# GLAD-RUC/FastEGNN

Measured on AMD Instinct MI355X. Metric: graphs/sec (fwd+bwd), Water-3D-like 100k-node frame, higher is better.
Workload: dtype f32; 1 GPU; cfg4 Water-3D-like frame (SURVEY 8d): uniform points, radius graph r=0.035 (mean degree ~19), gravity on; 4-layer FastEGNN H=64, fwd+loss+bwd, CSR build inside the step; nodes=100000, edges=1919172, graphs_per_batch=1, virtual_channels=16, layers=4, parallelism=1 GPU, launch=whole step replayed as one captured HIP graph

## Files before the change

### fastegnn_amd/csrc/common.h

```cpp
#pragma once
#include <hip/hip_runtime.h>
#include <stdint.h>

namespace fe {

typedef float f32x4 __attribute__((ext_vector_type(4)));

constexpr int H = 64;
constexpr int QXLD = 68;
constexpr int TS = 68;
constexpr int IMG = 4096;
constexpr int FEATW = 8;

struct Vec {
  f32x4 t[4];
};

__device__ __forceinline__ int lane_id() { return threadIdx.x & 63; }
__device__ __forceinline__ int wave_id() { return __builtin_amdgcn_readfirstlane((int)(threadIdx.x >> 6)); }
__device__ __forceinline__ int global_wave_id() { return (int)(blockIdx.x * (blockDim.x >> 6)) + wave_id(); }

__device__ __forceinline__ float sigmoid_f(float z) { return __builtin_amdgcn_rcpf(1.0f + __expf(-z)); }
__device__ __forceinline__ float silu_f(float z) { return z * sigmoid_f(z); }
__device__ __forceinline__ float dsilu_f(float z) {
// ... 399 lines not shown
  for (int p = 0; p < 3; ++p) fr[0][p] = ip[p * 512];
  __builtin_amdgcn_sched_group_barrier(0x100, 3, 0);
#pragma unroll
  for (int g = 0; g < 8; ++g) {
    const int s = g >> 2, t = g & 3, cb = g & 1;
    if (g + 1 < 8) {
      const int sn = (g + 1) >> 2, tn = (g + 1) & 3;
#pragma unroll
      for (int p = 0; p < 3; ++p) fr[cb ^ 1][p] = ip[p * 512 + (tn * 2 + sn) * 64];
      __builtin_amdgcn_sched_group_barrier(0x100, 3, 0);
    }
    const bf16x8 ah = __builtin_bit_cast(bf16x8, fr[cb][0]), am = __builtin_bit_cast(bf16x8, fr[cb][1]),
                 al = __builtin_bit_cast(bf16x8, fr[cb][2]);
    const bf16x8 xh = __builtin_bit_cast(bf16x8, in.p[0][s]);
    const bf16x8 xm = __builtin_bit_cast(bf16x8, in.p[1][s]);
    const bf16x8 xl = __builtin_bit_cast(bf16x8, in.p[2][s]);
    acc.t[t] = __builtin_amdgcn_mfma_f32_16x16x32_bf16(al, xh, acc.t[t], 0, 0, 0);
    acc.t[t] = __builtin_amdgcn_mfma_f32_16x16x32_bf16(am, xm, acc.t[t], 0, 0, 0);
    acc.t[t] = __builtin_amdgcn_mfma_f32_16x16x32_bf16(ah, xl, acc.t[t], 0, 0, 0);
    acc.t[t] = __builtin_amdgcn_mfma_f32_16x16x32_bf16(am, xh, acc.t[t], 0, 0, 0);
    acc.t[t] = __builtin_amdgcn_mfma_f32_16x16x32_bf16(ah, xm, acc.t[t], 0, 0, 0);
    acc.t[t] = __builtin_amdgcn_mfma_f32_16x16x32_bf16(ah, xh, acc.t[t], 0, 0, 0);
    __builtin_amdgcn_sched_group_barrier(0x008, 6, 0);
  }
  __builtin_amdgcn_sched_barrier(0);
#endif
}
__device__ __forceinline__ void gemm64_x3(const unsigned *img3, const Vec &in, Vec &acc) { gemm64_x3(img3, vsplit(in), acc); }

__device__ __forceinline__ void gemm64_x3_t2(const unsigned *img3, const Vec &v, Vec &acc) {
  const u32x4 *ip = reinterpret_cast<const u32x4 *>(img3) + lane_id();
#pragma unroll
  for (int s = 0; s < 2; ++s) {
    float x[8];
    u32x4 ph, pm;
#pragma unroll
    for (int e = 0; e < 8; ++e) x[e] = v.t[2 * s + (e >> 2)][e & 3];
#pragma unroll
    for (int w = 0; w < 4; ++w) {
      ph[w] = part_pack(x[2 * w], x[2 * w + 1]);
      pm[w] = part_pack(x[2 * w], x[2 * w + 1]);
    }
    const bf16x8 xh = __builtin_bit_cast(bf16x8, ph), xm = __builtin_bit_cast(bf16x8, pm);
#pragma unroll
    for (int t = 0; t < 4; ++t) {
      const bf16x8 ah = __builtin_bit_cast(bf16x8, ip[(t * 2 + s) * 64]);
      const bf16x8 am = __builtin_bit_cast(bf16x8, ip[512 + (t * 2 + s) * 64]);
      const bf16x8 al = __builtin_bit_cast(bf16x8, ip[1024 + (t * 2 + s) * 64]);
      acc.t[t] = __builtin_amdgcn_mfma_f32_16x16x32_bf16(al, xh, acc.t[t], 0, 0, 0);
      acc.t[t] = __builtin_amdgcn_mfma_f32_16x16x32_bf16(am, xm, acc.t[t], 0, 0, 0);
      acc.t[t] = __builtin_amdgcn_mfma_f32_16x16x32_bf16(am, xh, acc.t[t], 0, 0, 0);
      acc.t[t] = __builtin_amdgcn_mfma_f32_16x16x32_bf16(ah, xm, acc.t[t], 0, 0, 0);
      acc.t[t] = __builtin_amdgcn_mfma_f32_16x16x32_bf16(ah, xh, acc.t[t], 0, 0, 0);
    }
  }
}

typedef float f32x2 __attribute__((ext_vector_type(2)));
typedef __bf16 bf16x2 __attribute__((ext_vector_type(2)));
__device__ __forceinline__ unsigned pack_rne(float x0, float x1) {
  return __builtin_bit_cast(unsigned, __builtin_convertvector(f32x2{x0, x1}, bf16x2));
}
__device__ __forceinline__ float round_bf(float x) { return (float)(__bf16)x; }
__host__ __device__ __forceinline__ float round_bf_host(float x) {
  unsigned u = __builtin_bit_cast(unsigned, x);
  u = (u + 0x7fffu + ((u >> 16) & 1u)) & 0xffff0000u;
  return __builtin_bit_cast(float, u);
}
struct BfOp {
  u32x4 p[2];
};
__device__ __forceinline__ BfOp vpack_bf(const Vec &v) {
  BfOp B;
#pragma unroll
  for (int s = 0; s < 2; ++s)
#pragma unroll
    for (int w = 0; w < 4; ++w) {
      const int e = 2 * w;
      B.p[s][w] = pack_rne(v.t[2 * s + (e >> 2)][e & 3], v.t[2 * s + ((e + 1) >> 2)][(e + 1) & 3]);
    }
  return B;
}
__device__ __forceinline__ Vec vround(const Vec &v) { return vmap(v, [](float z) { return round_bf(z); }); }
__device__ __forceinline__ void gemm64_b1(const unsigned *img3, const BfOp &in, Vec &acc) {
  const u32x4 *ip = reinterpret_cast<const u32x4 *>(img3) + lane_id();
#pragma unroll
  for (int s = 0; s < 2; ++s) {
    const bf16x8 x = __builtin_bit_cast(bf16x8, in.p[s]);
#pragma unroll
    for (int t = 0; t < 4; ++t)
      acc.t[t] = __builtin_amdgcn_mfma_f32_16x16x32_bf16(__builtin_bit_cast(bf16x8, ip[(t * 2 + s) * 64]), x, acc.t[t], 0, 0, 0);
  }
}

constexpr int RM_RS = 144;
constexpr int RM_PART = 64 * RM_RS;
constexpr int RM_BYTES = 3 * RM_PART;
constexpr int RM_WORDS = RM_BYTES / 4;
typedef unsigned u32x2 __attribute__((ext_vector_type(2)));
typedef short s16x4 __attribute__((ext_vector_type(4)));
__device__ __forceinline__ u32x2 lds_tr_read(const char *p) {
  return __builtin_bit_cast(u32x2, __builtin_amdgcn_ds_read_tr16_b64_v4i16(
                                       (__attribute__((address_space(3))) s16x4 *)(p)));
}
template <bool TR>
__device__ __forceinline__ bf16x8 rm_frag(const char *img, int part, int t, int s) {
  const int l = lane_id(), i = l & 15, q = l >> 4;
  u32x2 lo, hi;
  if constexpr (TR) {
    const char *p = img + part * RM_PART + (32 * s + 4 * q + (i >> 2)) * RM_RS + (16 * t + 4 * (i & 3)) * 2;
    lo = lds_tr_read(p);
    hi = lds_tr_read(p + 16 * RM_RS);
  } else {
    const char *p = img + part * RM_PART + (16 * t + i) * RM_RS + (32 * s + 4 * q) * 2;
#ifdef FE_RM_READ2
    lo = *reinterpret_cast<const u32x2 *>(p);
    hi = *reinterpret_cast<const u32x2 *>(p + 32);
#else
    typedef __attribute__((address_space(3))) const volatile u32x2 *lds_vu32x2;
    lo = *(lds_vu32x2)(p);
    hi = *(lds_vu32x2)(p + 32);
#endif
  }
  return __builtin_bit_cast(bf16x8, u32x4{lo[0], lo[1], hi[0], hi[1]});
}
template <bool TR, bool PIPE = true>
__device__ __forceinline__ void gemm64_x3_rm(const char *img, const Split &in, Vec &acc) {
#ifdef FE_NO_GEMM_PIPE
  constexpr bool pipe = false;
#else
  constexpr bool pipe = PIPE;
#endif
  if constexpr (!pipe) {
#pragma unroll
  for (int s = 0; s < 2; ++s)
#pragma unroll
    for (int t = 0; t < 4; ++t) {
      const bf16x8 ah = rm_frag<TR>(img, 0, t, s), am = rm_frag<TR>(img, 1, t, s), al = rm_frag<TR>(img, 2, t, s);
      const bf16x8 xh = __builtin_bit_cast(bf16x8, in.p[0][s]);
      const bf16x8 xm = __builtin_bit_cast(bf16x8, in.p[1][s]);
      const bf16x8 xl = __builtin_bit_cast(bf16x8, in.p[2][s]);
      acc.t[t] = __builtin_amdgcn_mfma_f32_16x16x32_bf16(al, xh, acc.t[t], 0, 0, 0);
      acc.t[t] = __builtin_amdgcn_mfma_f32_16x16x32_bf16(am, xm, acc.t[t], 0, 0, 0);
      acc.t[t] = __builtin_amdgcn_mfma_f32_16x16x32_bf16(ah, xl, acc.t[t], 0, 0, 0);
      acc.t[t] = __builtin_amdgcn_mfma_f32_16x16x32_bf16(am, xh, acc.t[t], 0, 0, 0);
      acc.t[t] = __builtin_amdgcn_mfma_f32_16x16x32_bf16(ah, xm, acc.t[t], 0, 0, 0);
      acc.t[t] = __builtin_amdgcn_mfma_f32_16x16x32_bf16(ah, xh, acc.t[t], 0, 0, 0);
    }
  } else {
  __builtin_amdgcn_sched_barrier(0);
  bf16x8 fr[2][3];
#pragma unroll
  for (int p = 0; p < 3; ++p) fr[0][p] = rm_frag<TR>(img, p, 0, 0);
  __builtin_amdgcn_sched_group_barrier(0x100, 6, 0);
#pragma unroll
  for (int g = 0; g < 8; ++g) {
    const int s = g >> 2, t = g & 3, cb = g & 1;
    if (g + 1 < 8) {
#pragma unroll
      for (int p = 0; p < 3; ++p) fr[cb ^ 1][p] = rm_frag<TR>(img, p, (g + 1) & 3, (g + 1) >> 2);
      __builtin_amdgcn_sched_group_barrier(0x100, 6, 0);
    }
    const bf16x8 ah = fr[cb][0], am = fr[cb][1], al = fr[cb][2];
    const bf16x8 xh = __builtin_bit_cast(bf16x8, in.p[0][s]);
    const bf16x8 xm = __builtin_bit_cast(bf16x8, in.p[1][s]);
    const bf16x8 xl = __builtin_bit_cast(bf16x8, in.p[2][s]);
// ... 586 lines not shown
```

### fastegnn_amd/csrc/misc.hip

```cpp
#include <cstdlib>
#include "kernels.h"

namespace fe {

__global__ void embed_fwd_kernel(const float *nf, int N, int nfd, const float *W, const float *b, float *h) {
  long idx = (long)blockIdx.x * blockDim.x + threadIdx.x;
  if (idx >= (long)N * H) return;
  int n = (int)(idx >> 6), o = (int)(idx & 63);
  float acc = b[o];
  for (int a = 0; a < nfd; ++a) acc += nf[(size_t)n * nfd + a] * W[o * nfd + a];
  h[idx] = acc;
}
__global__ void dgrad_small_kernel(const float *G, long N, int kf, const float *W, int ldw, int c0, float *g_in, int accumulate) {
  long idx = (long)blockIdx.x * blockDim.x + threadIdx.x;
  if (idx >= N * kf) return;
  long n = idx / kf;
  int a = (int)(idx % kf);
  float acc = 0.f;
  for (int o = 0; o < H; ++o) acc += G[(size_t)n * H + o] * W[(size_t)o * ldw + c0 + a];
  g_in[idx] = accumulate ? g_in[idx] + acc : acc;
}

__global__ void virtual_init_kernel(const float *vnf, int B, int C, float *HvT) {
  long idx = (long)blockIdx.x * blockDim.x + threadIdx.x;
// ... 146 lines not shown
      for (int ti = 0; ti < 4; ++ti) {
        if (want_bias && !rnd) bsum[ti] += av[ti];
#pragma unroll
        for (int tk = 0; tk < 4; ++tk)
          acc[ti][tk] = __builtin_amdgcn_mfma_f32_16x16x4f32(av[ti], bv[tk], acc[ti][tk], 0, 0, 0);
      }
    }
  }
}

#ifndef FE_WG_DEPTH
#define FE_WG_DEPTH 2
#endif
__device__ __forceinline__ void wg_accumulate_direct(const float *G, const float *T, int ldg, int ldt, long m_first, long m1,
                                                     int step, bool want_bias, bool rnd, f32x4 (&acc)[4][4], float (&bsum)[4]) {
  constexpr int D = FE_WG_DEPTH;
  const int l = lane_id(), i = l & 15, k = l >> 4;
  float gv[D][16], tv[D][16];
  unsigned og[4], ot[4];
#pragma unroll
  for (int s = 0; s < 4; ++s) {
    og[s] = ((unsigned)(4 * s + k) * (unsigned)ldg + (unsigned)i) * 4u;
    ot[s] = ((unsigned)(4 * s + k) * (unsigned)ldt + (unsigned)i) * 4u;
  }
  auto issue = [&](int slot, long m) {
    const char *gb = reinterpret_cast<const char *>(G + (size_t)m * ldg);
    const char *tb = reinterpret_cast<const char *>(T + (size_t)m * ldt);
    const bool full = m + 16 <= m1;
#pragma unroll
    for (int s = 0; s < 4; ++s) {
      const bool ok = full || m + 4 * s + k < m1;
      const unsigned a = ok ? og[s] : (unsigned)i * 4u, b = ok ? ot[s] : (unsigned)i * 4u;
#pragma unroll
      for (int t = 0; t < 4; ++t) {
        gv[slot][4 * s + t] = *reinterpret_cast<const float *>(gb + a + 64u * t);
        tv[slot][4 * s + t] = *reinterpret_cast<const float *>(tb + b + 64u * t);
      }
    }
  };
  auto consume = [&](int slot, long m) {
    const bool full = m + 16 <= m1;
#pragma unroll
    for (int s = 0; s < 4; ++s) {
      float av[4], bv[4];
      const bool ok = full || m + 4 * s + k < m1;
#pragma unroll
      for (int t = 0; t < 4; ++t) {
        av[t] = ok ? gv[slot][4 * s + t] : 0.f;
        bv[t] = ok ? tv[slot][4 * s + t] : 0.f;
      }
      if (rnd) {
#pragma unroll
        for (int t = 0; t < 4; ++t) {
          if (want_bias) bsum[t] += av[t];
          av[t] = round_bf(av[t]);
          bv[t] = round_bf(bv[t]);
        }
      }
#pragma unroll
      for (int ti = 0; ti < 4; ++ti) {
        if (want_bias && !rnd) bsum[ti] += av[ti];
#pragma unroll
        for (int tk = 0; tk < 4; ++tk)
          acc[ti][tk] = __builtin_amdgcn_mfma_f32_16x16x4f32(av[ti], bv[tk], acc[ti][tk], 0, 0, 0);
      }
    }
  };
  long m = m_first;
#pragma unroll
  for (int d = 0; d < D; ++d)
    if (m + (long)d * step < m1) issue(d, m + (long)d * step);
  while (m < m1) {
#pragma unroll
    for (int d = 0; d < D; ++d) {
      if (m < m1) {
        consume(d, m);
        if (m + (long)D * step < m1) issue(d, m + (long)D * step);
        m += step;
      }
    }
  }
}

struct WgParts { u32x4 p[3]; };
template <bool BF>
__device__ __forceinline__ WgParts wg_split8(const float (&x)[8]) {
  WgParts P;
  if constexpr (BF) {
#pragma unroll
    for (int w = 0; w < 4; ++w) P.p[0][w] = pack_rne(x[2 * w], x[2 * w + 1]);
    P.p[1] = P.p[2] = u32x4{0u, 0u, 0u, 0u};
  } else {
    float y[8];
#pragma unroll
    for (int e = 0; e < 8; ++e) y[e] = x[e];
#pragma unroll
    for (int w = 0; w < 4; ++w) {
      P.p[0][w] = part_pack(y[2 * w], y[2 * w + 1]);
      P.p[1][w] = part_pack(y[2 * w], y[2 * w + 1]);
      P.p[2][w] = part_pack(y[2 * w], y[2 * w + 1]);
    }
  }
  return P;
}
template <bool BF>
__device__ __forceinline__ void wg_accumulate_x3(const float *G, const float *T, int ldg, int ldt, long m_first, long m1,
                                                 int step, bool want_bias, f32x4 (&acc)[4][4], float (&bsum)[4]) {
  const int l = lane_id(), i = l & 15, q = l >> 4;
  float gr[4][8], tr[4][8];
  unsigned og[8], ot[8];
#pragma unroll
  for (int e = 0; e < 8; ++e) {
    og[e] = ((unsigned)(8 * q + e) * (unsigned)ldg + (unsigned)i) * 4u;
    ot[e] = ((unsigned)(8 * q + e) * (unsigned)ldt + (unsigned)i) * 4u;
  }
  auto load_g = [&](long m) {
    const char *gb = reinterpret_cast<const char *>(G + (size_t)m * ldg);
    const bool full = m + 32 <= m1;
#pragma unroll
    for (int e = 0; e < 8; ++e) {
      const unsigned a = (full || m + 8 * q + e < m1) ? og[e] : (unsigned)i * 4u;
#pragma unroll
      for (int t = 0; t < 4; ++t) gr[t][e] = *reinterpret_cast<const float *>(gb + a + 64u * t);
    }
  };
  auto load_t = [&](long m, int t) {
    const char *tb = reinterpret_cast<const char *>(T + (size_t)m * ldt);
    const bool full = m + 32 <= m1;
#pragma unroll
    for (int e = 0; e < 8; ++e) {
      const unsigned a = (full || m + 8 * q + e < m1) ? ot[e] : (unsigned)i * 4u;
      tr[t][e] = *reinterpret_cast<const float *>(tb + a + 64u * t);
    }
  };
  long m = m_first;
  if (m < m1) {
    load_g(m);
#pragma unroll
    for (int t = 0; t < 4; ++t) load_t(m, t);
  }
  for (; m < m1; m += step) {
    const bool full = m + 32 <= m1;
    const bool more = m + step < m1;
    WgParts gp[4];
#pragma unroll
    for (int t = 0; t < 4; ++t) {
      if (!full) {
#pragma unroll
        for (int e = 0; e < 8; ++e)
          if (m + 8 * q + e >= m1) gr[t][e] = 0.f;
      }
      if (want_bias) {
#pragma unroll
        for (int e = 0; e < 8; ++e) bsum[t] += gr[t][e];
      }
      gp[t] = wg_split8<BF>(gr[t]);
    }
    if (more) load_g(m + step);
#pragma unroll
    for (int tk = 0; tk < 4; ++tk) {
      if (!full) {
#pragma unroll
        for (int e = 0; e < 8; ++e)
          if (m + 8 * q + e >= m1) tr[tk][e] = 0.f;
      }
      const WgParts tp = wg_split8<BF>(tr[tk]);
      if (more) load_t(m + step, tk);
      const bf16x8 bh = __builtin_bit_cast(bf16x8, tp.p[0]), bm = __builtin_bit_cast(bf16x8, tp.p[1]),
                   bl = __builtin_bit_cast(bf16x8, tp.p[2]);
#pragma unroll
      for (int ti = 0; ti < 4; ++ti) {
        const bf16x8 ah = __builtin_bit_cast(bf16x8, gp[ti].p[0]);
        if constexpr (BF) {
          acc[ti][tk] = __builtin_amdgcn_mfma_f32_16x16x32_bf16(ah, bh, acc[ti][tk], 0, 0, 0);
        } else {
          const bf16x8 am = __builtin_bit_cast(bf16x8, gp[ti].p[1]), al = __builtin_bit_cast(bf16x8, gp[ti].p[2]);
          acc[ti][tk] = __builtin_amdgcn_mfma_f32_16x16x32_bf16(al, bh, acc[ti][tk], 0, 0, 0);
          acc[ti][tk] = __builtin_amdgcn_mfma_f32_16x16x32_bf16(am, bm, acc[ti][tk], 0, 0, 0);
          acc[ti][tk] = __builtin_amdgcn_mfma_f32_16x16x32_bf16(ah, bl, acc[ti][tk], 0, 0, 0);
          acc[ti][tk] = __builtin_amdgcn_mfma_f32_16x16x32_bf16(am, bh, acc[ti][tk], 0, 0, 0);
          acc[ti][tk] = __builtin_amdgcn_mfma_f32_16x16x32_bf16(ah, bm, acc[ti][tk], 0, 0, 0);
          acc[ti][tk] = __builtin_amdgcn_mfma_f32_16x16x32_bf16(ah, bh, acc[ti][tk], 0, 0, 0);
        }
      }
    }
  }
}

__global__ __launch_bounds__(256, FE_WG_OCC) void wgrad_tn_kernel(WgTable tab) {
#if defined(FE_WG_STAGED)
  __shared__ __attribute__((aligned(16))) float smem[4 * 2 * 16 * WTS];
#else
  __shared__ __attribute__((aligned(16))) float smem[4 * IMG];
#endif
  __shared__ float redb[H];
  float *red = smem;
  int jb = 0;
#pragma unroll 1
  while (jb + 1 < tab.n_jobs && (int)blockIdx.x >= tab.job[jb + 1].wg_begin) ++jb;
  const WgJob &a = tab.job[jb];
  const int local = blockIdx.x - a.wg_begin;
  int bidx = local % a.nb, split = local / a.nb;
#ifdef FE_WG_XCD
  if (a.nb > 1 && (a.nsplit & 7) == 0 && (a.wg_begin & 7) == 0) {
    const int xcd = local & 7, slot = local >> 3;
    bidx = slot % a.nb;
    split = xcd + 8 * (slot / a.nb);
  }
#endif
  const int l = lane_id(), i = l & 15, q = l >> 4, w = wave_id();
  const float *G = a.G + (size_t)bidx * a.sG;
  const float *T = a.T + (size_t)bidx * a.sT;
  const long m0 = (long)split * a.rows_per_wg;
  long m1 = m0 + a.rows_per_wg;
  if (m1 > a.M) m1 = a.M;
  if (threadIdx.x < H) redb[threadIdx.x] = 0.f;
  float *gt = smem + (w * 2 + 0) * 16 * WTS, *tt = smem + (w * 2 + 1) * 16 * WTS;
  f32x4 acc[4][4];
  float bsum[4] = {0.f, 0.f, 0.f, 0.f};
#pragma unroll
  for (int ti = 0; ti < 4; ++ti)
#pragma unroll
    for (int tk = 0; tk < 4; ++tk) acc[ti][tk] = f32x4{0.f, 0.f, 0.f, 0.f};
  const bool want_bias = a.db != nullptr;
#if defined(FE_WG_STAGED)
  wg_accumulate(G, T, a.ldg, a.ldt, m0 + 16 * w, m1, 64, want_bias, a.round != 0, gt, tt, acc, bsum);
#elif defined(FE_WG_F32)
  (void)gt; (void)tt;
  wg_accumulate_direct(G, T, a.ldg, a.ldt, m0 + 16 * w, m1, 64, want_bias, a.round != 0, acc, bsum);
#else
  (void)gt; (void)tt;
  if (a.round) wg_accumulate_x3<true>(G, T, a.ldg, a.ldt, m0 + 32 * w, m1, 128, want_bias, acc, bsum);
  else wg_accumulate_x3<false>(G, T, a.ldg, a.ldt, m0 + 32 * w, m1, 128, want_bias, acc, bsum);
#endif
#if defined(FE_WG_STAGED) || defined(FE_WG_ATOMIC_EPILOGUE)
  __syncthreads();
  for (int k = threadIdx.x; k < IMG; k += 256) red[k] = 0.f;
  __syncthreads();
#pragma unroll
  for (int ti = 0; ti < 4; ++ti)
#pragma unroll
    for (int tk = 0; tk < 4; ++tk)
#pragma unroll
      for (int r = 0; r < 4; ++r) atomicAdd(&red[(16 * ti + 4 * q + r) * H + 16 * tk + i], acc[ti][tk][r]);
#pragma unroll
  for (int ti = 0; ti < 4; ++ti) {
    float s = qsum(bsum[ti]);
    if (q == 0) atomicAdd(&redb[16 * ti + i], s);
  }
  __syncthreads();
  const size_t sidx = (size_t)a.slab_begin + (size_t)bidx * a.nsplit + split;
  f32x4 *dst = reinterpret_cast<f32x4 *>(tab.slab + sidx * IMG);
  const f32x4 *src = reinterpret_cast<const f32x4 *>(red);
  for (int k = threadIdx.x; k < IMG / 4; k += 256) dst[k] = src[k];
  if (threadIdx.x < H) tab.slab_b[sidx * H + threadIdx.x] = redb[threadIdx.x];
#else
  (void)red;
  f32x4 *part = reinterpret_cast<f32x4 *>(smem) + (size_t)w * (IMG / 4);
#pragma unroll
  for (int ti = 0; ti < 4; ++ti)
#pragma unroll
    for (int tk = 0; tk < 4; ++tk) part[(ti * 4 + tk) * 64 + l] = acc[ti][tk];
#pragma unroll
  for (int ti = 0; ti < 4; ++ti) {
    float s = qsum(bsum[ti]);
    if (q == 0) atomicAdd(&redb[16 * ti + i], s);
  }
// ... 583 lines not shown
```

### fastegnn_amd/csrc/virt_bwd.hip

```cpp
#include <cstdlib>
#include "stages.h"

namespace fe {

#ifdef FE_SAFE_WAITS
__device__ __forceinline__ int vb_ld(const int *p) { return __hip_atomic_load(p, __ATOMIC_ACQUIRE, __HIP_MEMORY_SCOPE_WORKGROUP); }
__device__ __forceinline__ void vb_st(int *p, int v) { __hip_atomic_store(p, v, __ATOMIC_RELEASE, __HIP_MEMORY_SCOPE_WORKGROUP); }
#else
__device__ __forceinline__ int vb_ld(const int *p) { return __atomic_load_n(p, __ATOMIC_RELAXED); }
__device__ __forceinline__ void vb_st(int *p, int v) { __atomic_store_n(p, v, __ATOMIC_RELAXED); }
#endif

#ifdef FE_STAMP
__device__ unsigned long long g_vb2_stamps[32];
#define VB2_T0() unsigned _vp = (unsigned)__builtin_amdgcn_s_memtime(); unsigned _va[12] = {0, 0, 0, 0, 0, 0, 0, 0, 0, 0, 0, 0};
#define VB2_T(i) { __builtin_amdgcn_sched_barrier(0); const unsigned _t = (unsigned)__builtin_amdgcn_s_memtime(); \
                   _va[i] += _t - _vp; _vp = _t; __builtin_amdgcn_sched_barrier(0); }
#define VB2_TEND(base) if (lane_id() == 0) { for (int _k = 0; _k < 12; ++_k) atomicAdd(&g_vb2_stamps[(base) + _k], (unsigned long long)_va[_k]); }
#elif defined(FE_ISA_MARK)
#define VB2_T0()
#define VB2_T(i) { __builtin_amdgcn_sched_barrier(0); asm volatile("; FE_MARK " #i); __builtin_amdgcn_sched_barrier(0); }
#define VB2_TEND(base)
#else
#define VB2_T0()
#define VB2_T(i)
#define VB2_TEND(base)
#endif

__device__ __forceinline__ Vec vb_dsilu_mul(const Vec &g, const Vec &z FE_ACT_P) {
  return vmap2(g, z, [=](float a, float b) { return a * dsilu_f(b FE_ACT_A); });
}
__device__ __forceinline__ Vec vb_mask(const Vec &v, bool keep) { return keep ? v : vzero(); }

struct VirtNodeArgs {
  const float *g_h_out, *npre, *g_x_out, *vel, *aggx, *wpack;
  float *wg_t3, *wg_gnp, *g_h, *g_aggm, *g_aggx, *g_svel, *g_sgrav;
  int N, flags, C;
  float g[3];
  float act_param = 0.f;
};
constexpr int VB_NODE_WAVES = 8;
template <bool BF>
__global__ __launch_bounds__(64 * VB_NODE_WAVES) void virt_bwd_node_kernel(VirtNodeArgs a) {
  constexpr int SM = BF ? GM_BF16 : GM_X3;
  extern __shared__ __attribute__((aligned(16))) float lds[];
  unsigned *img = reinterpret_cast<unsigned *>(lds);
  const bool rf = a.flags & FASTEGNN_F_RF;
  if (!rf) load_images_x3(img, wpack_x3(a.wpack, a.C, I_W3AT), 3);
  __syncthreads();
  const int l = lane_id(), j = l & 15, q = l >> 4;
  const int wave = global_wave_id(), nwaves = (gridDim.x * blockDim.x) >> 6;
  const int ntiles = (a.N + 15) >> 4;
  const bool clamp_aggx = a.flags & FASTEGNN_F_EGNN;
  for (int tile = wave; tile < ntiles; tile += nwaves) {
    const int n = tile * 16 + j;
    const bool valid = n < a.N;
    const int nc = valid ? n : a.N - 1;
    const Vec g_out = vb_mask(vload_row(a.g_h_out + (size_t)nc * H, q), valid);
    if (rf) {
      if (valid) {
        vstore_row(a.g_h + (size_t)n * H, q, g_out);
        vstore_row(a.g_aggm + (size_t)n * H, q, vzero());
      }
    } else {
      const Vec npre = vload_row(a.npre + (size_t)nc * H, q);
      Vec g_t3 = vzero();
      gemm_op<SM>(img, 2, make_operand<SM>(g_out), g_t3);
      const Vec g_np = vb_dsilu_mul(g_t3, npre FE_ACT(a));
      if (valid) {
        vstore_row(a.wg_t3 + (size_t)n * H, q, vsilu(npre FE_ACT(a)));
        vstore_row(a.wg_gnp + (size_t)n * H, q, g_np);
      }
      const typename OperandOf<SM>::type gop = make_operand<SM>(g_np);
      Vec g_h = (a.flags & FASTEGNN_F_RESIDUAL) ? g_out : vzero();
      gemm_op<SM>(img, 0, gop, g_h);
      if (valid) vstore_row(a.g_h + (size_t)n * H, q, g_h);
      Vec g_am = vzero();
      gemm_op<SM>(img, 1, gop, g_am);
      if (valid) vstore_row(a.g_aggm + (size_t)n * H, q, g_am);
    }
    if (valid && q == 0) {
      float sv = 0.f, sg = 0.f;
#pragma unroll
      for (int k = 0; k < 3; ++k) {
        const float gxn = a.g_x_out[(size_t)n * 3 + k];
        const bool pass = !clamp_aggx || fabsf(a.aggx[(size_t)n * 3 + k]) <= 100.f;
        a.g_aggx[(size_t)n * 3 + k] = pass ? gxn : 0.f;
        sv += gxn * a.vel[(size_t)n * 3 + k];
        sg += gxn * a.g[k];
      }
      a.g_svel[n] = sv;
      if (a.flags & FASTEGNN_F_GRAVITY) a.g_sgrav[n] = sg;
    }
  }
}

__global__ __launch_bounds__(256) void virt_bwd_node_skip_kernel(const float *g_x_out, const float *vel, float *g_h, float *g_aggm,
                                                                 float *g_aggx, float *g_svel, float *g_sgrav, int N, int flags,
                                                                 float g0, float g1, float g2) {
  const size_t i = (size_t)blockIdx.x * blockDim.x + threadIdx.x;
  if (i >= (size_t)N * (H / 4)) return;
  const f32x4 z = {0.f, 0.f, 0.f, 0.f};
  reinterpret_cast<f32x4 *>(g_h)[i] = z;
  reinterpret_cast<f32x4 *>(g_aggm)[i] = z;
  if ((i & (H / 4 - 1)) == 0) {
    const size_t n = i / (H / 4);
    const float g[3] = {g0, g1, g2};
    float sv = 0.f, sg = 0.f;
#pragma unroll
    for (int k = 0; k < 3; ++k) {
      const float gxn = g_x_out[n * 3 + k];
      g_aggx[n * 3 + k] = gxn;
      sv += gxn * vel[n * 3 + k];
      sg += gxn * g[k];
    }
    g_svel[n] = sv;
    if (flags & FASTEGNN_F_GRAVITY) g_sgrav[n] = sg;
  }
}

struct VirtGvArgs {
  const float *g_np, *g_poolV, *wpack;
  const int32_t *batch;
  float *Gv;
  size_t cstride;
  int N, C, ngroups, nranges;
};
constexpr int VB_GV_CH = 4;
constexpr int VB_GV_WAVES = 8;
template <bool BF>
__global__ __launch_bounds__(64 * VB_GV_WAVES) void virt_bwd_gv_kernel(VirtGvArgs a) {
  constexpr int SM = BF ? GM_BF16 : GM_X3;
  extern __shared__ __attribute__((aligned(16))) float lds[];
  char *img = reinterpret_cast<char *>(lds);
  const int grp = (int)blockIdx.x % a.ngroups, range = (int)blockIdx.x / a.ngroups;
  const int c0 = grp * VB_GV_CH, ncv = min(VB_GV_CH, a.C - c0);
  {
    const u32x4 *src = reinterpret_cast<const u32x4 *>(wpack_rm(a.wpack, a.C, RM_FIXED + c0));
    u32x4 *dst = reinterpret_cast<u32x4 *>(img);
    for (int i = threadIdx.x; i < ncv * (RM_BYTES / 16); i += blockDim.x) dst[i] = src[i];
  }
  __syncthreads();
  const int l = lane_id(), j = l & 15, q = l >> 4, wv = wave_id();
  const int ntiles = (a.N + 15) >> 4;
  const int t_lo = (int)((long)range * ntiles / a.nranges), t_hi = (int)((long)(range + 1) * ntiles / a.nranges);
  for (int tile = t_lo + wv; tile < t_hi; tile += VB_GV_WAVES) {
    const int n = tile * 16 + j;
    const bool valid = n < a.N;
    const int nc = valid ? n : a.N - 1;
    const int b = a.batch[nc];
    Vec g = vb_mask(vload_row(a.g_np + (size_t)nc * H, q), valid);
    if constexpr (BF) g = vround(g);
    const typename OperandOf<SM>::type op = make_operand<SM>(g);
    const float *pv = a.g_poolV + ((size_t)b * a.C + c0) * H;
#pragma unroll 1
    for (int k = 0; k < ncv; ++k) {
      Vec acc = vload_row(pv + (size_t)k * H, q);
      gemm_rm<SM, true>(img + k * RM_BYTES, op, acc);
#ifdef VB_GV_NT
      if (valid) {
        float *row = a.Gv + (size_t)(c0 + k) * a.cstride + (size_t)n * H;
#pragma unroll
        for (int t = 0; t < 4; ++t) __builtin_nontemporal_store(acc.t[t], reinterpret_cast<f32x4 *>(row + 16 * t + 4 * q));
      }
#else
      if (valid) vstore_row(a.Gv + (size_t)(c0 + k) * a.cstride + (size_t)n * H, q, acc);
#endif
    }
  }
}

#ifndef FE_VB_FLUSH
#define FE_VB_FLUSH 48
#endif
constexpr int VB_FLUSH = FE_VB_FLUSH;
// ... 1350 lines not shown
  } else {
    const int ngroups = cdiv(C, VB_GV_CH);
    int nranges = 256 / ngroups;
    const int max_ranges = cdiv(ntiles, VB_GV_WAVES);
    if (nranges > max_ranges) nranges = max_ranges;
    if (nranges < 1) nranges = 1;
    VirtGvArgs a{wg_gnp, L->g_poolV, L->wpack, L->batch, Gv, cstride, N, C, ngroups, nranges};
    const size_t lds = (size_t)VB_GV_CH * RM_BYTES;
    ProfScope ps(K_VIRT_BWD_GV, st);
    if (bf) hipLaunchKernelGGL((virt_bwd_gv_kernel<true>), dim3(ngroups * nranges), dim3(64 * VB_GV_WAVES), lds, st, a);
    else hipLaunchKernelGGL((virt_bwd_gv_kernel<false>), dim3(ngroups * nranges), dim3(64 * VB_GV_WAVES), lds, st, a);
  }
  if ((rc = check_launch("virt_bwd_gv_kernel"))) return rc;
  WgradBatch bb(L->wg_slab, st, bf, WG_SLABS / 2, WG_SLABS / 2);
  VirtBwd2Args A;
  A.f = make_virt_args(L);
  A.g_x_out = L->g_x_out; A.g_poolX = L->g_poolX; A.Gv = Gv;
  A.g_x = L->g_x; A.g_A = L->g_A; A.g_Bc = L->g_Bc; A.g_Zp = L->g_Zp;
  A.gA_part = gA_part; A.gx_part = gx_part; A.wg_v = wg_v; A.cstride = cstride;
  A.cons_scratch = gx_part + (size_t)256 * VB_FINE_TILES * (NGF - 1) * 16 * 4;
  A.ld_v0 = 2 * H + 1 + C;
  A.d_wxv2 = g[FASTEGNN_P_CRV2_W]; A.d_wxx2 = g[FASTEGNN_P_CVV2_W];
  A.d_wvr = g[FASTEGNN_P_VIRT0_W] + 2 * H;
  A.d_attw = g[FASTEGNN_P_ATTV_W]; A.d_attb = g[FASTEGNN_P_ATTV_B];
  A.NGF = NGF;
  int grid = ntiles < 256 ? ntiles : 256;
  if ((rc = bb.add_slabs(g[FASTEGNN_P_CRV0_W], H, 0, 1, g[FASTEGNN_P_CRV0_B], grid, &A.slab_x))) return rc;
  if ((rc = bb.add_slabs(g[FASTEGNN_P_CVV0_W], H, 0, 1, g[FASTEGNN_P_CVV0_B], grid, &A.slab_X))) return rc;
  if ((rc = bb.add_slabs(g[FASTEGNN_P_VIRT2_W], H, 0, 1, g[FASTEGNN_P_VIRT2_B], grid, &A.slab_v2))) return rc;
  A.slab = bb.tab.slab; A.slab_b = bb.tab.slab_b;
  static const int ring_want = getenv("FE_VB_RING") ? atoi(getenv("FE_VB_RING")) : 54;
  const int imgb = bf ? RM_BYTES : (GM_VIRT_BWD == GM_F16 ? rm_lds_bytes<GM_F16>() : RM_BYTES);
  A.ringA = ring_want / 10; A.ringB = ring_want % 10; A.nbank = 1;
  if (A.ringA < 2 || A.ringA > VB_MAXRING) A.ringA = 3;
  if (A.ringB < 2 || A.ringB > VB_MAXRING) A.ringB = 3;
  while (vb_lds_floats(C, A.ringA, A.ringB, 1, imgb) * sizeof(float) > 160 * 1024 && A.ringB > 2) --A.ringB;
  while (vb_lds_floats(C, A.ringA, A.ringB, 1, imgb) * sizeof(float) > 160 * 1024 && A.ringA > 2) --A.ringA;
  while (A.nbank < VB_MAXBANK && vb_lds_floats(C, A.ringA, A.ringB, A.nbank + 1, imgb) * sizeof(float) <= 160 * 1024) ++A.nbank;
  const size_t lds = vb_lds_floats(C, A.ringA, A.ringB, A.nbank, imgb) * sizeof(float);
  FE_REQUIRE(lds <= 160 * 1024, "virt_backward: LDS budget exceeded");
  {
    ProfScope ps(K_VIRT_BWD, st);
    const dim3 g3(grid), b3(64 * VB_WAVES);
    if (bf) { if (att) hipLaunchKernelGGL((virt_bwd_pc_kernel<true, true>), g3, b3, lds, st, A); else hipLaunchKernelGGL((virt_bwd_pc_kernel<true, false>), g3, b3, lds, st, A); }
    else { if (att) hipLaunchKernelGGL((virt_bwd_pc_kernel<false, true>), g3, b3, lds, st, A); else hipLaunchKernelGGL((virt_bwd_pc_kernel<false, false>), g3, b3, lds, st, A); }
  }
  if ((rc = check_launch("virt_bwd_pc_kernel"))) return rc;
  if (NGF > 1) {
    hipLaunchKernelGGL(virt_bwd_combine_kernel, dim3(grid * VB_FINE_TILES), dim3(256), 0, st, L->g_A, L->g_x, gA_part, gx_part, N, NGF - 1, grid);
    if ((rc = check_launch("virt_bwd_combine_kernel"))) return rc;
  }
  if (!rf && node) {
    const int ld_n0 = 2 * H + H * C + L->na;
    if ((rc = bb.add(wg_gnp, H, wg_v, H, N, g[FASTEGNN_P_NODE0_W], ld_n0, 2 * H, C, nullptr, C, 0, (long)cstride, 1))) return rc;
  }
  return bb.finish();
}

int virt_backward(const fastegnn_layer_t *L, hipStream_t st, WgradBatch *shared) {
  const bool egnn = has(L, FASTEGNN_F_EGNN), rf = has(L, FASTEGNN_F_RF);
  const bool node = egnn || rf || L->g_h_out;
  FE_REQUIRE(node || !L->g_HvT_out, "virt_backward: g_h_out is null and g_HvT_out is not (both null: no gradient for h / Hv; otherwise neither)");
  FE_REQUIRE(L->h && L->A && L->x && L->vel && L->aggm && (!node || L->npre) && L->batch && L->wpack && (!egnn || L->aggx),
             "virt_backward: null saved buffer");
  FE_REQUIRE((!node || L->g_h_out) && L->g_x_out && L->g_h && L->g_x && L->g_A && L->g_aggm && L->g_aggx && L->g_svel && L->wg_node &&
                 L->grads && L->wg_slab,
             "virt_backward: null gradient buffer");
  FE_REQUIRE(egnn ? L->C == 0
                  : (L->Bc && L->Z && (rf || !node || L->g_poolV) && L->g_poolX && L->g_Bc && L->g_Zp && L->wg_virt && L->C >= 1 && L->C <= 64),
             "virt_backward: virtual buffers null or virtual_channels outside [1,64] (0 with FASTEGNN_F_EGNN)");
  const int N = L->N, C = L->C;
  if (C > 0) {
    (void)hipMemsetAsync(L->g_Bc, 0, (size_t)L->B * C * H * sizeof(float), st);
    (void)hipMemsetAsync(L->g_Zp, 0, (size_t)L->B * 3 * C * sizeof(float), st);
  }
  if (N == 0) return check_launch("virt_backward(memset)");
  const bool bf = has(L, FASTEGNN_F_BF16);
  float *const *g = L->grads;
  FE_REQUIRE(!has(L, FASTEGNN_F_ATTENTION) || C == 0 || (g[FASTEGNN_P_ATTV_W] && g[FASTEGNN_P_ATTV_B]), "virt_backward: attention grads null");
  FE_REQUIRE(!has(L, FASTEGNN_F_GRAVITY) || L->g_sgrav, "virt_backward: g_sgrav null");
  float *wg_t3 = L->wg_node, *wg_gnp = L->wg_node + (size_t)N * H;
  const int ntiles = cdiv(N, 16);
  int rc;
  if (!node) {
    ProfScope ps(K_VIRT_BWD_NODE, st);
    hipLaunchKernelGGL(virt_bwd_node_skip_kernel, dim3(cdiv((long)N * (H / 4), 256)), dim3(256), 0, st, L->g_x_out, L->vel, L->g_h, L->g_aggm,
                       L->g_aggx, L->g_svel, L->g_sgrav, N, L->flags, L->gravity[0], L->gravity[1], L->gravity[2]);
  } else {
    VirtNodeArgs a{L->g_h_out, L->npre, L->g_x_out, L->vel, L->aggx, L->wpack, wg_t3, wg_gnp, L->g_h, L->g_aggm, L->g_aggx,
                   L->g_svel, L->g_sgrav, N, L->flags, C, {L->gravity[0], L->gravity[1], L->gravity[2]}, L->act_param};
    int grid = cdiv(ntiles, VB_NODE_WAVES);
    if (grid > 256) grid = 256;
    ProfScope ps(K_VIRT_BWD_NODE, st);
    if (bf) hipLaunchKernelGGL((virt_bwd_node_kernel<true>), dim3(grid), dim3(64 * VB_NODE_WAVES), 3 * IMG3 * sizeof(float), st, a);
    else hipLaunchKernelGGL((virt_bwd_node_kernel<false>), dim3(grid), dim3(64 * VB_NODE_WAVES), 3 * IMG3 * sizeof(float), st, a);
  }
  if ((rc = check_launch("virt_bwd_node_kernel"))) return rc;
  if (C == 0) {
    (void)hipMemcpyAsync(L->g_x, L->g_x_out, (size_t)N * 3 * sizeof(float), hipMemcpyDeviceToDevice, st);
    (void)hipMemsetAsync(L->g_A, 0, (size_t)N * H * sizeof(float), st);
    if ((rc = check_launch("virt_backward(C = 0)"))) return rc;
  } else if ((rc = virt_backward_channels(L, st, wg_gnp, node))) {
    return rc;
  }
  if (rf || !node) return FASTEGNN_OK;
  WgradBatch local(L->wg_slab, st);
  WgradBatch &wb = shared ? *shared : local;
  wb.round = bf;
  const int ld_n0 = 2 * H + H * C + L->na;
  if ((rc = wb.add(L->g_h_out, H, wg_t3, H, N, g[FASTEGNN_P_NODE2_W], H, 0, 1, g[FASTEGNN_P_NODE2_B]))) return rc;
  if ((rc = wb.add(wg_gnp, H, L->h, H, N, g[FASTEGNN_P_NODE0_W], ld_n0, 0, 1, g[FASTEGNN_P_NODE0_B]))) return rc;
  if ((rc = wb.add(wg_gnp, H, L->aggm, H, N, g[FASTEGNN_P_NODE0_W], ld_n0, H, 1, nullptr))) return rc;
  if (!shared && (rc = wb.finish())) return rc;
  if (L->na > 0) {
    if ((rc = launch_wgrad_small(wg_gnp, H, L->node_attr, L->na, L->na, N, g[FASTEGNN_P_NODE0_W], ld_n0, 2 * H + H * C, st))) return rc;
    if (L->g_node_attr)
      if ((rc = launch_dgrad_small(wg_gnp, N, L->na, L->params[FASTEGNN_P_NODE0_W], ld_n0, 2 * H + H * C, L->g_node_attr, 1, st))) return rc;
  }
  return FASTEGNN_OK;
}

}

#ifdef FE_STAMP
extern "C" int fastegnn_debug_read_vb2_stamps(unsigned long long *out, int reset) {
  if (hipMemcpyFromSymbol(out, HIP_SYMBOL(fe::g_vb2_stamps), sizeof(unsigned long long) * 32) != hipSuccess) return -1;
  if (reset) {
    unsigned long long z[32] = {0};
    (void)hipMemcpyToSymbol(HIP_SYMBOL(fe::g_vb2_stamps), z, sizeof(z));
  }
  return 0;
}
#endif

extern "C" int fastegnn_spin_timeouts(int reset) {
  int n = -1;
  if (hipMemcpyFromSymbol(&n, HIP_SYMBOL(fe::g_vbs_timeouts), sizeof(int)) != hipSuccess) return -1;
  if (reset) {
    const int z = 0;
    (void)hipMemcpyToSymbol(HIP_SYMBOL(fe::g_vbs_timeouts), &z, sizeof(int));
  }
  return n;
}
#ifdef FE_VBS_WATCHDOG
extern "C" int fastegnn_debug_read_vbs_dog(int *out, int reset) {
  if (hipMemcpyFromSymbol(out, HIP_SYMBOL(fe::g_vbs_dog), sizeof(int) * 64) != hipSuccess) return -1;
  if (reset) {
    int z[64] = {0};
    (void)hipMemcpyToSymbol(HIP_SYMBOL(fe::g_vbs_dog), z, sizeof(z));
  }
  return 0;
}
#endif
```

Baseline: 99.17 graphs/s.

## Fuse node MLP weight-gradient GEMMs into virtual backward node kernel

Result: no change. 98.72 graphs/s (median of 2 runs) (-0.5%).

```diff
diff --git a/fastegnn_amd/csrc/common.h b/fastegnn_amd/csrc/common.h
--- a/fastegnn_amd/csrc/common.h
+++ b/fastegnn_amd/csrc/common.h
@@ -505,6 +505,44 @@
   return B;
 }
 __device__ __forceinline__ Vec vround(const Vec &v) { return vmap(v, [](float z) { return round_bf(z); }); }
+
+struct WgParts { u32x4 p[3]; };
+template <bool BF>
+__device__ __forceinline__ WgParts wg_split8(const float (&x)[8]) {
+  WgParts P;
+  if constexpr (BF) {
+#pragma unroll
+    for (int w = 0; w < 4; ++w) P.p[0][w] = pack_rne(x[2 * w], x[2 * w + 1]);
+    P.p[1] = P.p[2] = u32x4{0u, 0u, 0u, 0u};
+  } else {
+    float y[8];
+#pragma unroll
+    for (int e = 0; e < 8; ++e) y[e] = x[e];
+#pragma unroll
+    for (int w = 0; w < 4; ++w) {
+      P.p[0][w] = part_pack(y[2 * w], y[2 * w + 1]);
+      P.p[1][w] = part_pack(y[2 * w], y[2 * w + 1]);
+      P.p[2][w] = part_pack(y[2 * w], y[2 * w + 1]);
+    }
+  }
+  return P;
+}
+template <bool BF>
+__device__ __forceinline__ void wg_mma_parts(f32x4 &acc, const WgParts &g, const WgParts &t) {
+  const bf16x8 ah = __builtin_bit_cast(bf16x8, g.p[0]), bh = __builtin_bit_cast(bf16x8, t.p[0]);
+  if constexpr (BF) {
+    acc = __builtin_amdgcn_mfma_f32_16x16x32_bf16(ah, bh, acc, 0, 0, 0);
+  } else {
+    const bf16x8 am = __builtin_bit_cast(bf16x8, g.p[1]), al = __builtin_bit_cast(bf16x8, g.p[2]);
+    const bf16x8 bm = __builtin_bit_cast(bf16x8, t.p[1]), bl = __builtin_bit_cast(bf16x8, t.p[2]);
+    acc = __builtin_amdgcn_mfma_f32_16x16x32_bf16(al, bh, acc, 0, 0, 0);
+    acc = __builtin_amdgcn_mfma_f32_16x16x32_bf16(am, bm, acc, 0, 0, 0);
+    acc = __builtin_amdgcn_mfma_f32_16x16x32_bf16(ah, bl, acc, 0, 0, 0);
+    acc = __builtin_amdgcn_mfma_f32_16x16x32_bf16(am, bh, acc, 0, 0, 0);
+    acc = __builtin_amdgcn_mfma_f32_16x16x32_bf16(ah, bm, acc, 0, 0, 0);
+    acc = __builtin_amdgcn_mfma_f32_16x16x32_bf16(ah, bh, acc, 0, 0, 0);
+  }
+}
 __device__ __forceinline__ void gemm64_b1(const unsigned *img3, const BfOp &in, Vec &acc) {
   const u32x4 *ip = reinterpret_cast<const u32x4 *>(img3) + lane_id();
 #pragma unroll
diff --git a/fastegnn_amd/csrc/misc.hip b/fastegnn_amd/csrc/misc.hip
--- a/fastegnn_amd/csrc/misc.hip
+++ b/fastegnn_amd/csrc/misc.hip
@@ -252,27 +252,6 @@
   }
 }
 
-struct WgParts { u32x4 p[3]; };
-template <bool BF>
-__device__ __forceinline__ WgParts wg_split8(const float (&x)[8]) {
-  WgParts P;
-  if constexpr (BF) {
-#pragma unroll
-    for (int w = 0; w < 4; ++w) P.p[0][w] = pack_rne(x[2 * w], x[2 * w + 1]);
-    P.p[1] = P.p[2] = u32x4{0u, 0u, 0u, 0u};
-  } else {
-    float y[8];
-#pragma unroll
-    for (int e = 0; e < 8; ++e) y[e] = x[e];
-#pragma unroll
-    for (int w = 0; w < 4; ++w) {
-      P.p[0][w] = part_pack(y[2 * w], y[2 * w + 1]);
-      P.p[1][w] = part_pack(y[2 * w], y[2 * w + 1]);
-      P.p[2][w] = part_pack(y[2 * w], y[2 * w + 1]);
-    }
-  }
-  return P;
-}
 template <bool BF>
 __device__ __forceinline__ void wg_accumulate_x3(const float *G, const float *T, int ldg, int ldt, long m_first, long m1,
                                                  int step, bool want_bias, f32x4 (&acc)[4][4], float (&bsum)[4]) {
@@ -336,23 +315,8 @@
       }
       const WgParts tp = wg_split8<BF>(tr[tk]);
       if (more) load_t(m + step, tk);
-      const bf16x8 bh = __builtin_bit_cast(bf16x8, tp.p[0]), bm = __builtin_bit_cast(bf16x8, tp.p[1]),
-                   bl = __builtin_bit_cast(bf16x8, tp.p[2]);
-#pragma unroll
-      for (int ti = 0; ti < 4; ++ti) {
-        const bf16x8 ah = __builtin_bit_cast(bf16x8, gp[ti].p[0]);
-        if constexpr (BF) {
-          acc[ti][tk] = __builtin_amdgcn_mfma_f32_16x16x32_bf16(ah, bh, acc[ti][tk], 0, 0, 0);
-        } else {
-          const bf16x8 am = __builtin_bit_cast(bf16x8, gp[ti].p[1]), al = __builtin_bit_cast(bf16x8, gp[ti].p[2]);
-          acc[ti][tk] = __builtin_amdgcn_mfma_f32_16x16x32_bf16(al, bh, acc[ti][tk], 0, 0, 0);
-          acc[ti][tk] = __builtin_amdgcn_mfma_f32_16x16x32_bf16(am, bm, acc[ti][tk], 0, 0, 0);
-          acc[ti][tk] = __builtin_amdgcn_mfma_f32_16x16x32_bf16(ah, bl, acc[ti][tk], 0, 0, 0);
-          acc[ti][tk] = __builtin_amdgcn_mfma_f32_16x16x32_bf16(am, bh, acc[ti][tk], 0, 0, 0);
-          acc[ti][tk] = __builtin_amdgcn_mfma_f32_16x16x32_bf16(ah, bm, acc[ti][tk], 0, 0, 0);
-          acc[ti][tk] = __builtin_amdgcn_mfma_f32_16x16x32_bf16(ah, bh, acc[ti][tk], 0, 0, 0);
-        }
-      }
+#pragma unroll
+      for (int ti = 0; ti < 4; ++ti) wg_mma_parts<BF>(acc[ti][tk], gp[ti], tp);
     }
   }
 }
diff --git a/fastegnn_amd/csrc/virt_bwd.hip b/fastegnn_amd/csrc/virt_bwd.hip
--- a/fastegnn_amd/csrc/virt_bwd.hip
+++ b/fastegnn_amd/csrc/virt_bwd.hip
@@ -1,4 +1,5 @@
 #include <cstdlib>
+#include <cstring>
 #include "stages.h"
 
 namespace fe {
@@ -38,9 +39,18 @@
   int N, flags, C;
   float g[3];
   float act_param = 0.f;
+  const float *h = nullptr, *aggm = nullptr;
+  float *slab = nullptr, *slab_b = nullptr;
+  int slab_n2 = 0, slab_n0h = 0, slab_n0a = 0, rounds = 0;
 };
 constexpr int VB_NODE_WAVES = 8;
-template <bool BF>
+constexpr int VBN_ROWS = 64;
+constexpr int VBN_STAGE = VBN_ROWS * TS;
+enum { VBN_GOUT = 0, VBN_T3, VBN_GNP, VBN_H, VBN_AGGM, VBN_OPERANDS };
+constexpr int VBN_FLUSH_ROUNDS = 6;
+constexpr int VBN_MAX_SLABS = 1536;
+inline size_t vbn_lds_bytes(bool wg) { return (3 * (size_t)IMG3 + (wg ? (size_t)VBN_OPERANDS * VBN_STAGE : 0)) * sizeof(float); }
+template <bool BF, bool WG>
 __global__ __launch_bounds__(64 * VB_NODE_WAVES) void virt_bwd_node_kernel(VirtNodeArgs a) {
   constexpr int SM = BF ? GM_BF16 : GM_X3;
   extern __shared__ __attribute__((aligned(16))) float lds[];
@@ -49,10 +59,19 @@
   if (!rf) load_images_x3(img, wpack_x3(a.wpack, a.C, I_W3AT), 3);
   __syncthreads();
   const int l = lane_id(), j = l & 15, q = l >> 4;
+  const int wv = wave_id();
   const int wave = global_wave_id(), nwaves = (gridDim.x * blockDim.x) >> 6;
   const int ntiles = (a.N + 15) >> 4;
   const bool clamp_aggx = a.flags & FASTEGNN_F_EGNN;
-  for (int tile = wave; tile < ntiles; tile += nwaves) {
+  const int t_end = WG ? a.rounds * nwaves : ntiles;
+  float *stage = lds + 3 * IMG3;
+  const int ti = wv >> 1, tk0 = 2 * (wv & 1);
+  f32x4 acc[3][2];
+  float bs[2] = {0.f, 0.f};
+#pragma unroll
+  for (int jb = 0; jb < 3; ++jb) acc[jb][0] = acc[jb][1] = f32x4{0.f, 0.f, 0.f, 0.f};
+  int round = 0;
+  for (int tile = wave; tile < t_end; tile += nwaves) {
     const int n = tile * 16 + j;
     const bool valid = n < a.N;
     const int nc = valid ? n : a.N - 1;
@@ -64,12 +83,18 @@
       }
     } else {
       const Vec npre = vload_row(a.npre + (size_t)nc * H, q);
+      Vec hv, av;
+      if constexpr (WG) {
+        hv = vb_mask(vload_row(a.h + (size_t)nc * H, q), valid);
+        av = vb_mask(vload_row(a.aggm + (size_t)nc * H, q), valid);
+      }
       Vec g_t3 = vzero();
       gemm_op<SM>(img, 2, make_operand<SM>(g_out), g_t3);
       const Vec g_np = vb_dsilu_mul(g_t3, npre FE_ACT(a));
+      const Vec t3 = vsilu(npre FE_ACT(a));
       if (valid) {
-        vstore_row(a.wg_t3 + (size_t)n * H, q, vsilu(npre FE_ACT(a)));
-        vstore_row(a.wg_gnp + (size_t)n * H, q, g_np);
+        if constexpr (!WG) vstore_row(a.wg_t3 + (size_t)n * H, q, t3);
+        if (!WG || a.wg_gnp) vstore_row(a.wg_gnp + (size_t)n * H, q, g_np);
       }
       const typename OperandOf<SM>::type gop = make_operand<SM>(g_np);
       Vec g_h = (a.flags & FASTEGNN_F_RESIDUAL) ? g_out : vzero();
@@ -78,6 +103,47 @@
       Vec g_am = vzero();
       gemm_op<SM>(img, 1, gop, g_am);
       if (valid) vstore_row(a.g_aggm + (size_t)n * H, q, g_am);
+      if constexpr (WG) {
+        auto park = [&](int op, const Vec &v) {
+          float *p = stage + op * VBN_STAGE + ((wv & 3) * 16 + j) * TS + 4 * q;
+#pragma unroll
+          for (int t = 0; t < 4; ++t) *reinterpret_cast<f32x4 *>(p + 16 * t) = v.t[t];
+        };
+        auto frag = [&](int op, int t, int s, float (&x)[8]) {
+          const float *p = stage + op * VBN_STAGE + (32 * s + 4 * q) * TS + 16 * t + j;
+#pragma unroll
+          for (int e = 0; e < 8; ++e) x[e] = p[(16 * (e >> 2) + (e & 3)) * TS];
+        };
+#pragma unroll 1
+        for (int ph = 0; ph < 2; ++ph) {
+          if ((wv >> 2) == ph) {
+            park(VBN_GOUT, g_out); park(VBN_T3, t3); park(VBN_GNP, g_np); park(VBN_H, hv); park(VBN_AGGM, av);
+          }
+          __syncthreads();
+#pragma unroll 1
+          for (int s = 0; s < VBN_ROWS / 32; ++s) {
+            float x[8];
+            frag(VBN_GOUT, ti, s, x);
+#pragma unroll
+            for (int e = 0; e < 8; ++e) bs[0] += x[e];
+            const WgParts go = wg_split8<BF>(x);
+            frag(VBN_GNP, ti, s, x);
+#pragma unroll
+            for (int e = 0; e < 8; ++e) bs[1] += x[e];
+            const WgParts gn = wg_split8<BF>(x);
+#pragma unroll
+            for (int u = 0; u < 2; ++u) {
+              frag(VBN_T3, tk0 + u, s, x);
+              wg_mma_parts<BF>(acc[0][u], go, wg_split8<BF>(x));
+              frag(VBN_H, tk0 + u, s, x);
+              wg_mma_parts<BF>(acc[1][u], gn, wg_split8<BF>(x));
+              frag(VBN_AGGM, tk0 + u, s, x);
+              wg_mma_parts<BF>(acc[2][u], gn, wg_split8<BF>(x));
+            }
+          }
+          __syncthreads();
+        }
+      }
     }
     if (valid && q == 0) {
       float sv = 0.f, sg = 0.f;
@@ -91,6 +157,29 @@
       }
       a.g_svel[n] = sv;
       if (a.flags & FASTEGNN_F_GRAVITY) a.g_sgrav[n] = sg;
+    }
+    if constexpr (WG) {
+      ++round;
+      if (round % VBN_FLUSH_ROUNDS == 0 || round == a.rounds) {
+        const size_t sl = (size_t)((round - 1) / VBN_FLUSH_ROUNDS) * gridDim.x + blockIdx.x;
+        const int first[3] = {a.slab_n2, a.slab_n0h, a.slab_n0a};
+#pragma unroll
+        for (int jb = 0; jb < 3; ++jb) {
+          float *dst = a.slab + ((size_t)first[jb] + sl) * IMG;
+#pragma unroll
+          for (int u = 0; u < 2; ++u) {
+#pragma unroll
+            for (int r = 0; r < 4; ++r) dst[(16 * ti + 4 * q + r) * H + 16 * (tk0 + u) + j] = acc[jb][u][r];
+            acc[jb][u] = f32x4{0.f, 0.f, 0.f, 0.f};
+          }
+        }
+        const float s0 = qsum(bs[0]), s1 = qsum(bs[1]);
+        if ((wv & 1) == 0 && q == 0) {
+          a.slab_b[((size_t)a.slab_n2 + sl) * H + 16 * ti + j] = s0;
+          a.slab_b[((size_t)a.slab_n0h + sl) * H + 16 * ti + j] = s1;
+        }
+        bs[0] = bs[1] = 0.f;
+      }
     }
   }
 }
@@ -1607,6 +1696,9 @@
   float *wg_t3 = L->wg_node, *wg_gnp = L->wg_node + (size_t)N * H;
   const int ntiles = cdiv(N, 16);
   int rc;
+  WgradBatch local(L->wg_slab, st);
+  WgradBatch &wb = shared ? *shared : local;
+  bool in_kernel = false;
   if (!node) {
     ProfScope ps(K_VIRT_BWD_NODE, st);
     hipLaunchKernelGGL(virt_bwd_node_skip_kernel, dim3(cdiv((long)N * (H / 4), 256)), dim3(256), 0, st, L->g_x_out, L->vel, L->g_h, L->g_aggm,
@@ -1616,9 +1708,29 @@
                    L->g_svel, L->g_sgrav, N, L->flags, C, {L->gravity[0], L->gravity[1], L->gravity[2]}, L->act_param};
     int grid = cdiv(ntiles, VB_NODE_WAVES);
     if (grid > 256) grid = 256;
+    const int rounds = cdiv(ntiles, grid * VB_NODE_WAVES), nflush = cdiv(rounds, VBN_FLUSH_ROUNDS);
+    const char *sw = getenv("FASTEGNN_NODE_WGRAD_TN");
+    in_kernel = !rf && !(sw && *sw && strcmp(sw, "0") != 0) && g[FASTEGNN_P_NODE2_W] && g[FASTEGNN_P_NODE0_W] &&
+                3 * grid * nflush <= VBN_MAX_SLABS;
+    if (in_kernel) {
+      const int ld_n0 = 2 * H + H * C + L->na;
+      a.h = L->h; a.aggm = L->aggm; a.rounds = rounds;
+      if (C == 0 && L->na == 0) a.wg_gnp = nullptr;
+      if ((rc = wb.add_slabs(g[FASTEGNN_P_NODE2_W], H, 0, 1, g[FASTEGNN_P_NODE2_B], grid * nflush, &a.slab_n2))) return rc;
+      if ((rc = wb.add_slabs(g[FASTEGNN_P_NODE0_W], ld_n0, 0, 1, g[FASTEGNN_P_NODE0_B], grid * nflush, &a.slab_n0h))) return rc;
+      if ((rc = wb.add_slabs(g[FASTEGNN_P_NODE0_W], ld_n0, H, 1, nullptr, grid * nflush, &a.slab_n0a))) return rc;
+      a.slab = wb.tab.slab; a.slab_b = wb.tab.slab_b;
+    }
+    const dim3 g3(grid), b3(64 * VB_NODE_WAVES);
+    const size_t lds = vbn_lds_bytes(in_kernel);
     ProfScope ps(K_VIRT_BWD_NODE, st);
-    if (bf) hipLaunchKernelGGL((virt_bwd_node_kernel<true>), dim3(grid), dim3(64 * VB_NODE_WAVES), 3 * IMG3 * sizeof(float), st, a);
-    else hipLaunchKernelGGL((virt_bwd_node_kernel<false>), dim3(grid), dim3(64 * VB_NODE_WAVES), 3 * IMG3 * sizeof(float), st, a);
+    if (in_kernel) {
+      if (bf) hipLaunchKernelGGL((virt_bwd_node_kernel<true, true>), g3, b3, lds, st, a);
+      else hipLaunchKernelGGL((virt_bwd_node_kernel<false, true>), g3, b3, lds, st, a);
+    } else {
+      if (bf) hipLaunchKernelGGL((virt_bwd_node_kernel<true, false>), g3, b3, lds, st, a);
+      else hipLaunchKernelGGL((virt_bwd_node_kernel<false, false>), g3, b3, lds, st, a);
+    }
   }
   if ((rc = check_launch("virt_bwd_node_kernel"))) return rc;
   if (C == 0) {
@@ -1629,13 +1741,13 @@
     return rc;
   }
   if (rf || !node) return FASTEGNN_OK;
-  WgradBatch local(L->wg_slab, st);
-  WgradBatch &wb = shared ? *shared : local;
   wb.round = bf;
   const int ld_n0 = 2 * H + H * C + L->na;
-  if ((rc = wb.add(L->g_h_out, H, wg_t3, H, N, g[FASTEGNN_P_NODE2_W], H, 0, 1, g[FASTEGNN_P_NODE2_B]))) return rc;
-  if ((rc = wb.add(wg_gnp, H, L->h, H, N, g[FASTEGNN_P_NODE0_W], ld_n0, 0, 1, g[FASTEGNN_P_NODE0_B]))) return rc;
-  if ((rc = wb.add(wg_gnp, H, L->aggm, H, N, g[FASTEGNN_P_NODE0_W], ld_n0, H, 1, nullptr))) return rc;
+  if (!in_kernel) {
+    if ((rc = wb.add(L->g_h_out, H, wg_t3, H, N, g[FASTEGNN_P_NODE2_W], H, 0, 1, g[FASTEGNN_P_NODE2_B]))) return rc;
+    if ((rc = wb.add(wg_gnp, H, L->h, H, N, g[FASTEGNN_P_NODE0_W], ld_n0, 0, 1, g[FASTEGNN_P_NODE0_B]))) return rc;
+    if ((rc = wb.add(wg_gnp, H, L->aggm, H, N, g[FASTEGNN_P_NODE0_W], ld_n0, H, 1, nullptr))) return rc;
+  }
   if (!shared && (rc = wb.finish())) return rc;
   if (L->na > 0) {
     if ((rc = launch_wgrad_small(wg_gnp, H, L->node_attr, L->na, L->na, N, g[FASTEGNN_P_NODE0_W], ld_n0, 2 * H + H * C, st))) return rc;
```
